# MECLabTUDA/Lifelong-nnUNet

Hardware: AMD Instinct MI355X
Metric: 3D patches/sec (whole node) + mean Dice vs ref, 5-level 3D Generic_UNet training step (higher is better)
Workload: dtype f16 (fp32 accumulate, fp32 master weights)

## Files before the change

lifelong-nnunet_amd/csrc/norm_act.hip:

```cpp
#include "igemm_common.h"

namespace {

constexpr int NT = 256;
typedef float float2v __attribute__((ext_vector_type(2)));
constexpr int MAX_BLOCKS = 1024;
constexpr int UNR = 4;

__device__ __forceinline__ half8 ld8(const half_t* p, int nt) {
    return nt ? __builtin_nontemporal_load(reinterpret_cast<const half8*>(p)) : *reinterpret_cast<const half8*>(p);
}
__device__ __forceinline__ void st8(half_t* p, const half8& v, int nt) {
    if (nt) __builtin_nontemporal_store(v, reinterpret_cast<half8*>(p));
    else *reinterpret_cast<half8*>(p) = v;
}
int in_nt_flag() {
    static int v = -1;
    if (v < 0) { const char* e = getenv("LNN_IN_NT"); v = (e && e[0] == '1') ? 1 : 0; }
    return v;
}

struct RowMap {
    int C8, VPB, c8, vl;
    bool active;
};
__device__ __forceinline__ RowMap row_map(int C) {
    RowMap r;
    r.C8 = C >> 3;
    r.VPB = NT / r.C8;
    r.c8 = threadIdx.x % r.C8;
    r.vl = threadIdx.x / r.C8;
    r.active = r.vl < r.VPB;
    return r;
}

__device__ __forceinline__ long vrange_len(long V, const RowMap& rm) {
    const long per = (V + gridDim.x - 1) / gridDim.x;
    return (per + rm.VPB - 1) / rm.VPB * rm.VPB;
}
__device__ __forceinline__ long vrange_begin(long V, const RowMap& rm) { return (long)blockIdx.x * vrange_len(V, rm); }
__device__ __forceinline__ long vrange_end(long V, const RowMap& rm) {
    const long e = vrange_begin(V, rm) + vrange_len(V, rm);
    return e < V ? e : V;
}

template <int NA, typename Sink>
__device__ __forceinline__ void block_channel_reduce(const RowMap& rm, int C, float (&part)[NA][8], float* red, Sink sink) {
    constexpr int W = NA * 8 + 1;
    __syncthreads();
    if (rm.active) {
#pragma unroll
        for (int a = 0; a < NA; ++a)
#pragma unroll
            for (int e = 0; e < 8; ++e) red[threadIdx.x * W + a * 8 + e] = part[a][e];
    }
    __syncthreads();
    for (int o = threadIdx.x; o < NA * C; o += NT) {
        const int a = o / C, c = o % C, c8 = c >> 3, e = c & 7;
        float s = 0.f;
        for (int vl = 0; vl < rm.VPB; ++vl) s += red[(vl * rm.C8 + c8) * W + a * 8 + e];
        sink(a, c, s);
    }
}

__global__ __launch_bounds__(NT) void in_stats_kernel(const half_t* __restrict__ y, long V, int C, float* pws) {
    __shared__ float red[NT * 17];
    const RowMap rm = row_map(C);
    const int n = blockIdx.y;
    const half_t* yn = y + (long)n * V * C;
    float part[2][8];
#pragma unroll
    for (int e = 0; e < 8; ++e) part[0][e] = part[1][e] = 0.f;
    if (rm.active) {
        const long end = vrange_end(V, rm), step = rm.VPB;
        long v = vrange_begin(V, rm) + rm.vl;
        const half_t* yp = yn + rm.c8 * 8;
        for (; v + (UNR - 1) * step < end; v += UNR * step) {
            half8 x[UNR];
#pragma unroll
            for (int u = 0; u < UNR; ++u) x[u] = *reinterpret_cast<const half8*>(yp + (v + u * step) * C);
#pragma unroll
            for (int u = 0; u < UNR; ++u)
#pragma unroll
                for (int e = 0; e < 8; ++e) {
                    const float f = (float)x[u][e];
                    part[0][e] += f;
                    part[1][e] += f * f;
                }
        }
        for (; v < end; v += step) {
            const half8 x = *reinterpret_cast<const half8*>(yp + v * C);
#pragma unroll
            for (int e = 0; e < 8; ++e) {
                const float f = (float)x[e];
                part[0][e] += f;
                part[1][e] += f * f;
            }
        }
    }
    block_channel_reduce<2>(rm, C, part, red, [&](int a, int c, float s) {
        pws[(((long)a * gridDim.x + blockIdx.x) * gridDim.y + n) * C + c] = s;
    });
}

constexpr int FSL = 64, FEB = 256 / FSL;
template <int SL>
__device__ __forceinline__ double slice_sum(const float* p, long stride, int nparts, int sl) {
    double acc = 0;
    int b = sl;
    for (; b + 15 * SL < nparts; b += 16 * SL) {
        float v[16];
#pragma unroll
        for (int k = 0; k < 16; ++k) v[k] = p[(long)(b + k * SL) * stride];
#pragma unroll
        for (int k = 0; k < 16; k += 4) acc += ((double)v[k] + (double)v[k + 1]) + ((double)v[k + 2] + (double)v[k + 3]);
    }
    for (; b + 3 * SL < nparts; b += 4 * SL) {
        const float a0 = p[(long)b * stride], a1 = p[(long)(b + SL) * stride], a2 = p[(long)(b + 2 * SL) * stride],
                    a3 = p[(long)(b + 3 * SL) * stride];
        acc += ((double)a0 + (double)a1) + ((double)a2 + (double)a3);
    }
    for (; b < nparts; b += SL) acc += (double)p[(long)b * stride];
    return acc;
}
template <int SL, int J>
__device__ __forceinline__ void reduce_slices(double (&s)[J], double* red) {
    constexpr int EB = 256 / SL;
    const int ii = threadIdx.x % EB, sl = threadIdx.x / EB;
    __syncthreads();
#pragma unroll
    for (int j = 0; j < J; ++j) red[j * 256 + threadIdx.x] = s[j];
    __syncthreads();
    if constexpr (SL > 16) {
        if (sl < 16) {
#pragma unroll
            for (int j = 0; j < J; ++j)
                for (int k = sl + 16; k < SL; k += 16) s[j] += red[j * 256 + k * EB + ii];
        }
        __syncthreads();
        if (sl < 16) {
#pragma unroll
            for (int j = 0; j < J; ++j) red[j * 256 + threadIdx.x] = s[j];
        }
        __syncthreads();
    }
    if (sl == 0) {
#pragma unroll
        for (int j = 0; j < J; ++j)
#pragma unroll
            for (int k = 1; k < 16; ++k) s[j] += red[j * 256 + k * EB + ii];
    }
}

__global__ void in_stats_finalize_kernel(const float* pws, int nblk, int NC, long V, float eps, float* mean, float* rstd) {
    __shared__ double red[2 * 256];
    const int ii = threadIdx.x % FEB, sl = threadIdx.x / FEB;
    const int i = blockIdx.x * FEB + ii;
    double t[2] = {0, 0};
    if (i < NC) {
        t[0] = slice_sum<FSL>(pws + i, NC, nblk, sl);
        t[1] = slice_sum<FSL>(pws + (long)nblk * NC + i, NC, nblk, sl);
    }
    reduce_slices<FSL, 2>(t, red);
    if (i >= NC || sl != 0) return;
    const double m = t[0] / (double)V;
    double var = t[1] / (double)V - m * m;
    if (var < 0) var = 0;
    mean[i] = (float)m;
    rstd[i] = (float)(1.0 / sqrt(var + (double)eps));
}

__global__ __launch_bounds__(NT) void in_lrelu_fwd_kernel(const half_t* __restrict__ y, half_t* __restrict__ z, int ld_z,
                                                          long V, int C, const float* __restrict__ mean,
                                                          const float* __restrict__ rstd, const float* __restrict__ gamma,
                                                          const float* __restrict__ beta, float slope, int nt) {
    const RowMap rm = row_map(C);
    if (!rm.active) return;
    const int n = blockIdx.y;
    float sc[8], sh[8];
#pragma unroll
    for (int e = 0; e < 8; ++e) {
        const int c = rm.c8 * 8 + e;
        sc[e] = gamma[c] * rstd[n * C + c];
        sh[e] = beta[c] - mean[n * C + c] * sc[e];
    }
    const half_t* yn = y + (long)n * V * C;
    half_t* zn = z + (long)n * V * ld_z;
    auto apply = [&](const half8& x) {
        half8 o;
#pragma unroll
        for (int e = 0; e < 8; ++e) {
            const float t = (float)x[e] * sc[e] + sh[e];
            o[e] = (half_t)(t > 0.f ? t : t * slope);
        }
        return o;
    };
    const long end = vrange_end(V, rm), step = rm.VPB;
    long v = vrange_begin(V, rm) + rm.vl;
    const half_t* yp = yn + rm.c8 * 8;
    half_t* zp = zn + rm.c8 * 8;
    for (; v + (UNR - 1) * step < end; v += UNR * step) {
        half8 x[UNR];
#pragma unroll
// ... 41 lines not shown
            const float zf = (float)o[e];
#pragma unroll
            for (int k = 0; k < KB; ++k) pk[k] += zf * w[k][e];
        }
        if (z) *reinterpret_cast<half8*>(zp + v * ld_z) = o;
        for (int m = 1; m < rm.C8; m <<= 1) {
#pragma unroll
            for (int k = 0; k < KB; ++k) pk[k] += __shfl_xor(pk[k], m, 64);
        }
        if (rm.c8 == 0) {
#pragma unroll
            for (int k = 0; k < KB; ++k)
                if (KT > 0 || k < K) {
                    if (stage) stage[k * (UNR * 64)] = pk[k];
                    else ln[(long)k * V + v] = pk[k];
                }
        }
    };
    long v = vrange_begin(V, rm) + rm.vl;
    if constexpr (STAGED) {
        const long run = (long)UNR * step;
        long base = vrange_begin(V, rm);
        int it = 0;
        for (; base + run <= end; base += run, ++it) {
            float* buf = lg + (it & 1) * (SEG_KMAX * UNR * 64);
            half8 x[UNR];
#pragma unroll
            for (int u = 0; u < UNR; ++u) x[u] = *reinterpret_cast<const half8*>(yp + (base + rm.vl + u * step) * C);
#pragma unroll
            for (int u = 0; u < UNR; ++u) one(x[u], base + rm.vl + u * step, buf + u * step + rm.vl);
            __syncthreads();
            const int q4 = (int)(run >> 2);
            for (int t = threadIdx.x; t < K * q4; t += NT) {
                const int k = t / q4, j = t - k * q4;
                *reinterpret_cast<floatx4*>(ln + (long)k * V + base + 4 * j) = *reinterpret_cast<const floatx4*>(buf + k * (UNR * 64) + 4 * j);
            }
        }
        v = base + rm.vl;
    } else {
        for (; v + (UNR - 1) * step < end; v += UNR * step) {
            half8 x[UNR];
#pragma unroll
            for (int u = 0; u < UNR; ++u) x[u] = *reinterpret_cast<const half8*>(yp + (v + u * step) * C);
#pragma unroll
            for (int u = 0; u < UNR; ++u) one(x[u], v + u * step, nullptr);
        }
    }
    for (; v < end; v += step) one(*reinterpret_cast<const half8*>(yp + v * C), v, nullptr);
}

__global__ __launch_bounds__(NT) void in_lrelu_bwd_reduce_kernel(const half_t* __restrict__ y, const half_t* __restrict__ dz,
                                                                 int ld_dz, long V, int C, const float* __restrict__ mean,
                                                                 const float* __restrict__ rstd, const float* __restrict__ gamma,
                                                                 const float* __restrict__ beta, float slope, float* pws, int nt) {
    __shared__ float red[NT * 17];
    const RowMap rm = row_map(C);
    const int n = blockIdx.y;
    float part[2][8];
#pragma unroll
    for (int e = 0; e < 8; ++e) part[0][e] = part[1][e] = 0.f;
    if (rm.active) {
        float mu[8], rs[8], ga[8], be[8];
#pragma unroll
        for (int e = 0; e < 8; ++e) {
            const int c = rm.c8 * 8 + e;
            mu[e] = mean[n * C + c]; rs[e] = rstd[n * C + c]; ga[e] = gamma[c]; be[e] = beta[c];
        }
        const half_t* yn = y + (long)n * V * C;
        const half_t* dzn = dz + (long)n * V * ld_dz;
        auto accum = [&](const half8& x, const half8& d) {
#pragma unroll
            for (int e = 0; e < 8; ++e) {
                const float xh = ((float)x[e] - mu[e]) * rs[e];
                const float pre = ga[e] * xh + be[e];
                const float g = (float)d[e] * (pre > 0.f ? 1.f : slope);
                part[0][e] += g;
                part[1][e] += g * xh;
            }
        };
        const long end = vrange_end(V, rm), step = rm.VPB;
        long v = vrange_begin(V, rm) + rm.vl;
        const half_t* yp = yn + rm.c8 * 8;
        const half_t* dp = dzn + rm.c8 * 8;
        constexpr int U2 = UNR / 2;
        for (; v + (U2 - 1) * step < end; v += U2 * step) {
            half8 x[U2], d[U2];
#pragma unroll
            for (int u = 0; u < U2; ++u) {
                x[u] = *reinterpret_cast<const half8*>(yp + (v + u * step) * C);
                d[u] = *reinterpret_cast<const half8*>(dp + (v + u * step) * ld_dz);
            }
#pragma unroll
            for (int u = 0; u < U2; ++u) accum(x[u], d[u]);
        }
        for (; v < end; v += step)
            accum(*reinterpret_cast<const half8*>(yp + v * C), *reinterpret_cast<const half8*>(dp + v * ld_dz));
    }
    block_channel_reduce<2>(rm, C, part, red, [&](int a, int c, float s) {
        pws[(((long)a * gridDim.x + blockIdx.x) * gridDim.y + n) * C + c] = s;
    });
}

__device__ __forceinline__ void in_bwd_sums_block(const float* pws, int nblk, int N, int C, int blk, double* red, double* ws,
                                                  float* dgamma, float* dbeta, float unscale, const float* raw_mean = nullptr,
                                                  const float* raw_rstd = nullptr) {
    const int ii = threadIdx.x % FEB, sl = threadIdx.x / FEB;
    const int c = blk * FEB + ii, NC = N * C;
    double g0 = 0, g1 = 0;
    for (int n = 0; n < N; n += 2) {
        const bool two = n + 1 < N;
        double o[4] = {0, 0, 0, 0};
        if (c < C) {
            const float* p0 = pws + n * C + c;
            o[0] = slice_sum<FSL>(p0, NC, nblk, sl);
            o[1] = slice_sum<FSL>(p0 + (long)nblk * NC, NC, nblk, sl);
            if (two) {
                o[2] = slice_sum<FSL>(p0 + C, NC, nblk, sl);
                o[3] = slice_sum<FSL>(p0 + C + (long)nblk * NC, NC, nblk, sl);
            }
        }
        reduce_slices<FSL, 4>(o, red);
        if (c < C && sl == 0) {
            const long i0 = (long)n * C + c;
            if (raw_mean) {
                o[1] = (double)raw_rstd[i0] * (o[1] - (double)raw_mean[i0] * o[0]);
                if (two) o[3] = (double)raw_rstd[i0 + C] * (o[3] - (double)raw_mean[i0 + C] * o[2]);
            }
            ws[i0 * 3 + 0] = o[0]; ws[i0 * 3 + 1] = o[1];
            g0 += o[0]; g1 += o[1];
            if (two) {
                ws[(i0 + C) * 3 + 0] = o[2]; ws[(i0 + C) * 3 + 1] = o[3];
                g0 += o[2]; g1 += o[3];
            }
        }
    }
    if (c >= C || sl != 0) return;
    if (dgamma) atomicAdd(dgamma + c, (float)(g1 * unscale));
    if (dbeta) atomicAdd(dbeta + c, (float)(g0 * unscale));
}
__global__ void in_lrelu_bwd_sums_kernel(const float* pws, int nblk, int NC, int C, double* ws, float* dgamma, float* dbeta,
                                         float unscale, const float* raw_mean, const float* raw_rstd) {
    __shared__ double red[4 * 256];
    in_bwd_sums_block(pws, nblk, NC / C, C, blockIdx.x, red, ws, dgamma, dbeta, unscale, raw_mean, raw_rstd);
}

template <bool DBIAS>
__global__ __launch_bounds__(NT) void in_lrelu_bwd_apply_kernel(half_t* __restrict__ y, const half_t* __restrict__ dz, int ld_dz,
                                                                long V, int C, const float* __restrict__ mean,
                                                                const float* __restrict__ rstd, const float* __restrict__ gamma,
                                                                const float* __restrict__ beta, float slope, const double* ws,
                                                                float* pws, int nt) {
    __shared__ float red[NT * 9];
    const RowMap rm = row_map(C);
// ... 58 lines not shown
    double t[1] = {i < N * C ? slice_sum<FSL>(pws + i, N * C, nblk, sl) : 0.0};
    reduce_slices<FSL, 1>(t, red);
    const double db = t[0];
    if (i >= N * C || sl != 0) return;
    const int c = i % C;
    (void)ws; (void)dgamma; (void)dbeta;
    if (dbias) atomicAdd(dbias + c, (float)(db * unscale));
}

template <int KT>
__device__ __forceinline__ void seg_dz(const float (&d)[KT], const float (&wr)[KT][8], const half8* prior, half8& dzh) {
#pragma unroll
    for (int e = 0; e < 8; ++e) {
        float o = 0.f;
#pragma unroll
        for (int k = 0; k < KT; ++k) o += d[k] * wr[k][e];
        if (prior) o += (float)(*prior)[e];
        dzh[e] = (half_t)o;
    }
}

template <int KT, bool QUAD>
struct DlFetch {
    float raw[QUAD ? 1 : KT];
    __device__ __forceinline__ void load(const float* __restrict__ dln, long V, long v) {
        if constexpr (QUAD) {
            const int kq = (int)(threadIdx.x & 3);
            raw[0] = dln[(long)(kq < KT ? kq : KT - 1) * V + v];
        } else {
#pragma unroll
            for (int k = 0; k < KT; ++k) raw[k] = dln[(long)k * V + v];
        }
    }
    __device__ __forceinline__ void get(float (&d)[KT]) const {
        if constexpr (QUAD) {
            const int r = __builtin_bit_cast(int, raw[0]);
            d[0] = __builtin_bit_cast(float, __builtin_amdgcn_mov_dpp(r, 0x00, 0xf, 0xf, true));
            if constexpr (KT > 1) d[1] = __builtin_bit_cast(float, __builtin_amdgcn_mov_dpp(r, 0x55, 0xf, 0xf, true));
            if constexpr (KT > 2) d[2] = __builtin_bit_cast(float, __builtin_amdgcn_mov_dpp(r, 0xaa, 0xf, 0xf, true));
            if constexpr (KT > 3) d[3] = __builtin_bit_cast(float, __builtin_amdgcn_mov_dpp(r, 0xff, 0xf, 0xf, true));
        } else {
#pragma unroll
            for (int k = 0; k < KT; ++k) d[k] = raw[k];
        }
    }
};

template <int KT, bool PRIOR, bool QUAD>
__global__ __launch_bounds__(NT, (KT <= 3 && !PRIOR && QUAD) ? 3 : 2) void in_lrelu_seg_bwd_reduce_kernel(const half_t* __restrict__ y, const half_t* __restrict__ dzp,
                                                                     int ld_dz, long V, int C, const float* __restrict__ mean,
                                                                     const float* __restrict__ rstd, const float* __restrict__ gamma,
                                                                     const float* __restrict__ beta, float slope,
                                                                     const float* __restrict__ segw, const float* __restrict__ dl,
                                                                     float* pws) {
    constexpr int NA = 2 + KT;
    __shared__ float red[NT * 17];
    const RowMap rm = row_map(C);
    const int n = blockIdx.y;
    float part[NA][8];
#pragma unroll
    for (int a = 0; a < NA; ++a)
#pragma unroll
        for (int e = 0; e < 8; ++e) part[a][e] = 0.f;
    if (rm.active) {
        float rs[8], nmr[8], sc[8], sh[8], wr[KT][8];
#pragma unroll
        for (int e = 0; e < 8; ++e) {
            const int c = rm.c8 * 8 + e;
            rs[e] = rstd[n * C + c];
            nmr[e] = -mean[n * C + c] * rs[e];
            sc[e] = gamma[c] * rs[e];
            sh[e] = beta[c] - mean[n * C + c] * sc[e];
#pragma unroll
            for (int k = 0; k < KT; ++k) wr[k][e] = segw[k * C + c];
        }
        const half_t* yp = y + (long)n * V * C + rm.c8 * 8;
        const half_t* dp = dzp + (long)n * V * ld_dz + rm.c8 * 8;
        const float* dln = dl + (long)n * KT * V;
        auto accum = [&](const half8& x, const half8& pr, const float (&d)[KT]) {
#pragma unroll
            for (int e = 0; e < 8; e += 2) {
                const float2v xf = {(float)x[e], (float)x[e + 1]};
                const float2v sc2 = {sc[e], sc[e + 1]}, sh2 = {sh[e], sh[e + 1]}, rs2 = {rs[e], rs[e + 1]}, nm2 = {nmr[e], nmr[e + 1]};
                const float2v t = xf * sc2 + sh2;
                const float2v sel = {t[0] > 0.f ? 1.f : slope, t[1] > 0.f ? 1.f : slope};
                const float2v z = t * sel;
                const float2v xh = xf * rs2 + nm2;
                float2v dz = {0.f, 0.f};
#pragma unroll
                for (int k = 0; k < KT; ++k) {
                    const float2v wk = {wr[k][e], wr[k][e + 1]};
                    dz += wk * d[k];
                }
                if (PRIOR) dz += float2v{(float)pr[e], (float)pr[e + 1]};
                const float2v g = dz * sel;
                float2v p0 = {part[0][e], part[0][e + 1]}, p1 = {part[1][e], part[1][e + 1]};
                p0 += g;
                p1 += g * xh;
                part[0][e] = p0[0]; part[0][e + 1] = p0[1];
                part[1][e] = p1[0]; part[1][e + 1] = p1[1];
#pragma unroll
                for (int k = 0; k < KT; ++k) {
                    float2v pk = {part[2 + k][e], part[2 + k][e + 1]};
                    pk += z * d[k];
                    part[2 + k][e] = pk[0]; part[2 + k][e + 1] = pk[1];
                }
            }
        };
        const long end = vrange_end(V, rm), step = rm.VPB;
        long v = vrange_begin(V, rm) + rm.vl;
        constexpr int U2 = (PRIOR || !QUAD) ? UNR / 2 : 3;
        for (; v + (U2 - 1) * step < end; v += U2 * step) {
            half8 x[U2], pr[U2];
            DlFetch<KT, QUAD> df[U2];
#pragma unroll
            for (int u = 0; u < U2; ++u) {
                x[u] = *reinterpret_cast<const half8*>(yp + (v + u * step) * C);
                if (PRIOR) pr[u] = *reinterpret_cast<const half8*>(dp + (v + u * step) * ld_dz);
                df[u].load(dln, V, v + u * step);
            }
#pragma unroll
            for (int u = 0; u < U2; ++u) {
                float d[KT];
                df[u].get(d);
                accum(x[u], pr[u], d);
            }
        }
        for (; v < end; v += step) {
            half8 pr;
            float d[KT];
            DlFetch<KT, QUAD> df;
            if (PRIOR) pr = *reinterpret_cast<const half8*>(dp + v * ld_dz);
            df.load(dln, V, v);
            df.get(d);
            accum(*reinterpret_cast<const half8*>(yp + v * C), pr, d);
        }
    }
    float* const pseg = pws + 2l * gridDim.x * gridDim.y * C;
#pragma unroll
    for (int a0 = 0; a0 < NA; a0 += 2) {
        float two[2][8];
#pragma unroll
        for (int e = 0; e < 8; ++e) {
            two[0][e] = part[a0][e];
            two[1][e] = a0 + 1 < NA ? part[a0 + 1 < NA ? a0 + 1 : a0][e] : 0.f;
        }
        block_channel_reduce<2>(rm, C, two, red, [&](int a, int c, float s) {
            const int aa = a0 + a;
            if (aa < 2) pws[(((long)aa * gridDim.x + blockIdx.x) * gridDim.y + n) * C + c] = s;
            else if (aa < NA) pseg[(((long)n * gridDim.x + blockIdx.x) * KT + (aa - 2)) * C + c] = s;
        });
    }
}

__global__ void in_lrelu_seg_bwd_sums_kernel(const float* pws, int nblk, int N, int C, int K, int nb_in, double* ws, float* dgamma,
                                             float* dbeta, float* dsegw, float unscale) {
    __shared__ double red[4 * 256];
    if ((int)blockIdx.x < nb_in) {
        in_bwd_sums_block(pws, nblk, N, C, blockIdx.x, red, ws, dgamma, dbeta, unscale);
        return;
    }
    const float* pseg = pws + 2l * nblk * N * C;
    const int ii = threadIdx.x % FEB, sl = threadIdx.x / FEB;
    const int i = (blockIdx.x - nb_in) * FEB + ii;
    double t[1] = {i < K * C ? slice_sum<FSL>(pseg + i, (long)K * C, nblk * N, sl) : 0.0};
    reduce_slices<FSL, 1>(t, red);
    if (sl == 0 && i < K * C) atomicAdd(dsegw + i, (float)(t[0] * unscale));
}

template <int KT, bool PRIOR, bool QUAD>
__global__ __launch_bounds__(NT) void in_lrelu_seg_bwd_apply_kernel(half_t* __restrict__ y, const half_t* __restrict__ dzp, int ld_dz,
                                                                    long V, int C, const float* __restrict__ mean,
                                                                    const float* __restrict__ rstd, const float* __restrict__ gamma,
                                                                    const float* __restrict__ beta, float slope,
                                                                    const float* __restrict__ segw, const float* __restrict__ dl,
                                                                    const double* ws) {
    const RowMap rm = row_map(C);
    if (!rm.active) return;
    const int n = blockIdx.y;
    float sc[8], sh[8], ca[8], cb[8], wr[KT][8];
    const float invV = 1.0f / (float)V;
#pragma unroll
    for (int e = 0; e < 8; ++e) {
        const int c = rm.c8 * 8 + e;
        const float rs = rstd[n * C + c], nmr = -mean[n * C + c] * rs;
        const float m1 = (float)(ws[((long)n * C + c) * 3 + 0] * (double)invV);
        const float m2 = (float)(ws[((long)n * C + c) * 3 + 1] * (double)invV);
        sc[e] = gamma[c] * rs;
        sh[e] = beta[c] - mean[n * C + c] * sc[e];
        ca[e] = -sc[e] * (m1 + nmr * m2);
        cb[e] = -sc[e] * rs * m2;
#pragma unroll
        for (int k = 0; k < KT; ++k) wr[k][e] = segw[k * C + c];
    }
    half_t* yp = y + (long)n * V * C + rm.c8 * 8;
    const half_t* dp = dzp + (long)n * V * ld_dz + rm.c8 * 8;
    const float* dln = dl + (long)n * KT * V;
    auto grad = [&](const half8& x, const half8& pr, const float (&d)[KT]) {
        half8 dzh, o;
        seg_dz<KT>(d, wr, PRIOR ? &pr : nullptr, dzh);
#pragma unroll
        for (int e = 0; e < 8; ++e) {
            const float xf = (float)x[e];
            const float t = xf * sc[e] + sh[e];
// ... 178 lines not shown
        }
        small_block_sum16(part, red, dtot);
        if (threadIdx.x < 64) {
            const double t = dtot[threadIdx.x];
            const int o = threadIdx.x >> 4, j = threadIdx.x & 15, c = blockIdx.x * 32 + o * 8 + (j & 7);
            bc[threadIdx.x] = (float)(t * (double)invV);
            gacc += t;
            if (c < C) ws[((long)n * C + c) * 3 + (j >> 3)] = t;
        }
        __syncthreads();
        if (chan_ok) {
            float m1[8], m2[8];
#pragma unroll
            for (int e = 0; e < 8; ++e) { m1[e] = bc[oc * 16 + e]; m2[e] = bc[oc * 16 + 8 + e]; }
            for (int r0 = rl; r0 < V; r0 += SU * SRL) {
                half8 xv[SU], gv[SU];
#pragma unroll
                for (int k = 0; k < SU; ++k) {
                    const int r = r0 + k * SRL, rc = r < V ? r : V - 1;
                    xv[k] = *reinterpret_cast<const half8*>(yn + rc * C);
                    gv[k] = *reinterpret_cast<const half8*>(dn + rc * ld_dz);
                }
#pragma unroll
                for (int k = 0; k < SU; ++k) {
                    half8 o;
#pragma unroll
                    for (int e = 0; e < 8; ++e) {
                        const float h = ((float)xv[k][e] - mu[e]) * rs[e];
                        const float pre = ga[e] * h + be[e];
                        const float gg = (float)gv[k][e] * (pre > 0.f ? 1.f : slope);
                        o[e] = (half_t)(ga[e] * rs[e] * (gg - m1[e] - h * m2[e]));
                    }
                    const int r = r0 + k * SRL;
                    if (r < V) *reinterpret_cast<half8*>(yn + r * C) = o;
                }
            }
        }
    }
    if (threadIdx.x < 64) {
        const int o = threadIdx.x >> 4, j = threadIdx.x & 15, c = blockIdx.x * 32 + o * 8 + (j & 7);
        if (c < C) {
            if (j < 8) { if (dbeta) atomicAdd(dbeta + c, (float)(gacc * unscale)); }
            else if (dgamma) atomicAdd(dgamma + c, (float)(gacc * unscale));
        }
    }
}

bool small_enabled() {
    static int v = -1;
    if (v < 0) { const char* e = getenv("LNN_IN_SMALL"); v = (e && e[0] == '0') ? 0 : 1; }
    return v != 0;
}

int blocks_for(long V, int C) {
    const int vpb = NT / (C / 8);
    long b = (V + (long)vpb * 8 - 1) / ((long)vpb * 8);
    if (b > MAX_BLOCKS) b = MAX_BLOCKS;
    if (b < 1) b = 1;
    return (int)b;
}

int check_common(const void* y, int N, long V, int C, const char* what) {
    LNN_REQUIRE(y != nullptr && lnn_aligned16(y), "%s: null/misaligned activation", what);
    LNN_REQUIRE(N > 0 && V > 0, "%s: bad dims", what);
    LNN_REQUIRE(C >= 8 && C % 8 == 0 && C <= 2048, "%s: channel count %d must be a multiple of 8 in [8, 2048]", what, C);
    return LNN_OK;
}

}

extern "C" int lnn_instnorm_small_volume(void) { return SMALL_V; }

int lnn_launch_in_small_fwd(hipStream_t s, const void* y, void* z, int ld_z, int N, long V, int C, float eps, const float* gamma,
                            const float* beta, float slope, float* mean, float* rstd) {
    if (int e = check_common(y, N, V, C, "lnn_conv3d_fwd_in_lrelu(norm)")) return e;
    LNN_REQUIRE(V <= SMALL_V, "lnn_conv3d_fwd_in_lrelu(norm): %ld voxels per sample exceed the single-launch limit %d", V, SMALL_V);
    LNN_REQUIRE(z != nullptr && lnn_aligned16(z) && ld_z >= C && ld_z % 8 == 0, "lnn_conv3d_fwd_in_lrelu(norm): bad z / ld_z");
    LNN_REQUIRE(mean && rstd && gamma && beta, "lnn_conv3d_fwd_in_lrelu(norm): null parameter");
    const dim3 grid(lnn_cdiv(C, 32), N);
    hipLaunchKernelGGL(in_small_fwd_kernel, grid, dim3(SNT), 0, s, (const half_t*)y, (half_t*)z, ld_z, (int)V, C, eps, gamma, beta, slope,
                       mean, rstd);
    LNN_CHECK_LAUNCH("lnn_conv3d_fwd_in_lrelu(norm)");
    return LNN_OK;
}

int lnn_launch_in_small_bwd(hipStream_t s, void* y, const void* dz, int ld_dz, int N, long V, int C, const float* mean, const float* rstd,
                            const float* gamma, const float* beta, float slope, double* ws, float* dgamma, float* dbeta, float unscale) {
    LNN_REQUIRE(V <= SMALL_V, "lnn_instnorm_lrelu_bwd(small): %ld voxels per sample exceed the single-launch limit %d", V, SMALL_V);
    hipLaunchKernelGGL(in_small_bwd_kernel, dim3(lnn_cdiv(C, 32)), dim3(SNT), 0, s, (half_t*)y, (const half_t*)dz, ld_dz, N, (int)V, C, mean,
                       rstd, gamma, beta, slope, ws, dgamma, dbeta, unscale);
    LNN_CHECK_LAUNCH("lnn_instnorm_lrelu_bwd(small)");
    return LNN_OK;
}

int lnn_launch_in_stats_finalize(hipStream_t s, const float* pws, int nslots, int N, int C, long V, float eps, float* mean, float* rstd) {
    hipLaunchKernelGGL(in_stats_finalize_kernel, dim3(lnn_cdiv(N * C, FEB)), dim3(256), 0, s, pws, nslots, N * C, V, eps, mean, rstd);
    LNN_CHECK_LAUNCH("lnn_instnorm_stats(finalize, fused partials)");
    return LNN_OK;
}

int lnn_launch_in_bwd_sums_raw(hipStream_t s, const float* pws, int nslots, int N, int C, const float* mean, const float* rstd,
                               double* ws, float* dgamma, float* dbeta, float unscale) {
    hipLaunchKernelGGL(in_lrelu_bwd_sums_kernel, dim3(lnn_cdiv(C, FEB)), dim3(256), 0, s, pws, nslots, N * C, C, ws, dgamma, dbeta,
                       unscale, mean, rstd);
    LNN_CHECK_LAUNCH("lnn_conv3d_dgrad_in_bwd_sums(sums)");
    return LNN_OK;
}

extern "C" size_t lnn_instnorm_ws_doubles(int N, int C) { return (size_t)N * C * 3 + (size_t)MAX_BLOCKS * N * C; }

extern "C" int lnn_instnorm_stats(lnn_stream_t s_, const void* y, int N, long V, int C, float eps, float* mean, float* rstd,
                                  double* ws) {
    hipStream_t s = (hipStream_t)s_;
    if (int e = check_common(y, N, V, C, "lnn_instnorm_stats")) return e;
    LNN_REQUIRE(mean && rstd && ws, "lnn_instnorm_stats: null output/workspace");
    float* pws = reinterpret_cast<float*>(ws + (size_t)N * C * 3);
    const int nblk = blocks_for(V, C);
    hipLaunchKernelGGL(in_stats_kernel, dim3(nblk, N), dim3(NT), 0, s, (const half_t*)y, V, C, pws);
    LNN_CHECK_LAUNCH("lnn_instnorm_stats");
    hipLaunchKernelGGL(in_stats_finalize_kernel, dim3(lnn_cdiv(N * C, FEB)), dim3(256), 0, s, pws, nblk, N * C, V, eps, mean, rstd);
    LNN_CHECK_LAUNCH("lnn_instnorm_stats(finalize)");
    return LNN_OK;
}

extern "C" int lnn_instnorm_lrelu_fwd(lnn_stream_t s_, const void* y, void* z, int ld_z, int N, long V, int C,
                                      const float* mean, const float* rstd, const float* gamma, const float* beta,
                                      float slope) {
    hipStream_t s = (hipStream_t)s_;
    if (int e = check_common(y, N, V, C, "lnn_instnorm_lrelu_fwd")) return e;
    LNN_REQUIRE(z != nullptr && lnn_aligned16(z) && ld_z >= C && ld_z % 8 == 0, "lnn_instnorm_lrelu_fwd: bad z / ld_z");
    LNN_REQUIRE(mean && rstd && gamma && beta, "lnn_instnorm_lrelu_fwd: null parameter");
    hipLaunchKernelGGL(in_lrelu_fwd_kernel, dim3(blocks_for(V, C), N), dim3(NT), 0, s, (const half_t*)y, (half_t*)z, ld_z,
                       V, C, mean, rstd, gamma, beta, slope, in_nt_flag());
    LNN_CHECK_LAUNCH("lnn_instnorm_lrelu_fwd");
    return LNN_OK;
}

extern "C" int lnn_instnorm_lrelu_seg_fwd(lnn_stream_t s_, const void* y, void* z, int ld_z, int N, long V, int C, const float* mean,
                                          const float* rstd, const float* gamma, const float* beta, float slope,
                                          const float* seg_w, float* logits, int K) {
    hipStream_t s = (hipStream_t)s_;
    if (int e = check_common(y, N, V, C, "lnn_instnorm_lrelu_seg_fwd")) return e;
    LNN_REQUIRE(z == nullptr || (lnn_aligned16(z) && ld_z >= C && ld_z % 8 == 0), "lnn_instnorm_lrelu_seg_fwd: bad z / ld_z");
    LNN_REQUIRE(mean && rstd && gamma && beta && seg_w && logits, "lnn_instnorm_lrelu_seg_fwd: null parameter");
    const int C8 = C >> 3;
    LNN_REQUIRE(K >= 1 && K <= SEG_KMAX && (C8 & (C8 - 1)) == 0 && C8 <= 64,
                "lnn_instnorm_lrelu_seg_fwd: K=%d / C=%d unsupported (K <= %d, C/8 a power of two <= 64): use lnn_instnorm_lrelu_fwd + lnn_seg1x1_fwd",
                K, C, SEG_KMAX);
    static int want_staged = -1;
    if (want_staged < 0) { const char* e = getenv("LNN_SEG_FWD_STAGED"); want_staged = (e && e[0] == '1') ? 1 : 0; }
    const bool staged = want_staged && C8 >= 4 && (V & 3) == 0 && lnn_aligned16(logits);
#define LNN_SF(ST, KT) hipLaunchKernelGGL((in_lrelu_seg_fwd_kernel<ST, KT>), dim3(blocks_for(V, C), N), dim3(NT), 0, s, (const half_t*)y, \
                                         (half_t*)z, ld_z, V, C, mean, rstd, gamma, beta, slope, seg_w, logits, K)
    if (staged) LNN_SF(true, 0);
    else if (K == 1) LNN_SF(false, 1);
    else if (K == 2) LNN_SF(false, 2);
    else if (K == 3) LNN_SF(false, 3);
    else if (K == 4) LNN_SF(false, 4);
    else LNN_SF(false, 0);
#undef LNN_SF
    LNN_CHECK_LAUNCH("lnn_instnorm_lrelu_seg_fwd");
    return LNN_OK;
}

extern "C" int lnn_instnorm_lrelu_bwd(lnn_stream_t s_, void* y, const void* dz, int ld_dz, int N, long V, int C,
                                      const float* mean, const float* rstd, const float* gamma, const float* beta,
                                      float slope, float* dgamma, float* dbeta, float* dbias, float grad_unscale,
                                      double* ws) {
    hipStream_t s = (hipStream_t)s_;
    if (int e = check_common(y, N, V, C, "lnn_instnorm_lrelu_bwd")) return e;
    LNN_REQUIRE(dz != nullptr && lnn_aligned16(dz) && ld_dz >= C && ld_dz % 8 == 0, "lnn_instnorm_lrelu_bwd: bad dz / ld_dz");
    LNN_REQUIRE(mean && rstd && gamma && beta && ws, "lnn_instnorm_lrelu_bwd: null parameter");
    if (V <= SMALL_V && !dbias && small_enabled())
        return lnn_launch_in_small_bwd(s, y, dz, ld_dz, N, V, C, mean, rstd, gamma, beta, slope, ws, dgamma, dbeta, grad_unscale);
    float* pws = reinterpret_cast<float*>(ws + (size_t)N * C * 3);
    const int nblk = blocks_for(V, C);
    const dim3 grid(nblk, N);
    hipLaunchKernelGGL(in_lrelu_bwd_reduce_kernel, grid, dim3(NT), 0, s, (const half_t*)y, (const half_t*)dz, ld_dz, V, C,
                       mean, rstd, gamma, beta, slope, pws, in_nt_flag());
    LNN_CHECK_LAUNCH("lnn_instnorm_lrelu_bwd(reduce)");
    hipLaunchKernelGGL(in_lrelu_bwd_sums_kernel, dim3(lnn_cdiv(C, FEB)), dim3(256), 0, s, pws, nblk, N * C, C, ws, dgamma, dbeta,
                       grad_unscale, (const float*)nullptr, (const float*)nullptr);
    LNN_CHECK_LAUNCH("lnn_instnorm_lrelu_bwd(sums)");
    if (dbias) {
        hipLaunchKernelGGL((in_lrelu_bwd_apply_kernel<true>), grid, dim3(NT), 0, s, (half_t*)y, (const half_t*)dz, ld_dz, V, C, mean,
                           rstd, gamma, beta, slope, ws, pws, in_nt_flag());
        LNN_CHECK_LAUNCH("lnn_instnorm_lrelu_bwd(apply)");
        hipLaunchKernelGGL(in_lrelu_bwd_finalize_kernel, dim3(lnn_cdiv(N * C, FEB)), dim3(256), 0, s, ws, pws, nblk, N, C, dgamma,
                           dbeta, dbias, grad_unscale);
        LNN_CHECK_LAUNCH("lnn_instnorm_lrelu_bwd(finalize)");
    } else {
        hipLaunchKernelGGL((in_lrelu_bwd_apply_kernel<false>), grid, dim3(NT), 0, s, (half_t*)y, (const half_t*)dz, ld_dz, V, C, mean,
                           rstd, gamma, beta, slope, ws, pws, in_nt_flag());
        LNN_CHECK_LAUNCH("lnn_instnorm_lrelu_bwd(apply)");
    }
    return LNN_OK;
}

extern "C" size_t lnn_instnorm_lrelu_seg_bwd_ws_doubles(int N, int C) { return (size_t)N * C * 3 + (size_t)MAX_BLOCKS * N * C * 3; }

extern "C" int lnn_instnorm_lrelu_seg_bwd(lnn_stream_t s_, void* y, const void* dz_prior, int ld_dz, const float* seg_w,
                                          const float* dlogits, float* seg_dw, int K, int N, long V, int C, const float* mean,
                                          const float* rstd, const float* gamma, const float* beta, float slope, float* dgamma,
                                          float* dbeta, float grad_unscale, double* ws) {
    hipStream_t s = (hipStream_t)s_;
    if (int e = check_common(y, N, V, C, "lnn_instnorm_lrelu_seg_bwd")) return e;
    LNN_REQUIRE(dz_prior == nullptr || (lnn_aligned16(dz_prior) && ld_dz >= C && ld_dz % 8 == 0),
                "lnn_instnorm_lrelu_seg_bwd: bad dz_prior / ld_dz");
    LNN_REQUIRE(mean && rstd && gamma && beta && ws && seg_w && dlogits && seg_dw, "lnn_instnorm_lrelu_seg_bwd: null parameter");
    LNN_REQUIRE(K >= 1 && K <= 4, "lnn_instnorm_lrelu_seg_bwd: K=%d unsupported (1..4): use lnn_seg1x1_bwd + lnn_instnorm_lrelu_bwd", K);
    float* pws = reinterpret_cast<float*>(ws + (size_t)N * C * 3);
    const int nblk = blocks_for(V, C);
    const dim3 grid(nblk, N);
    const half_t* pr = (const half_t*)dz_prior;
    const int nb_in = lnn_cdiv(C, FEB);
#define LNN_SB(KT, PRIOR) do { if (C % 32 == 0) LNN_SBQ(KT, PRIOR, true); else LNN_SBQ(KT, PRIOR, false); } while (0)
#define LNN_SBQ(KT, PRIOR, QUAD)                                                                                                     \
    do {                                                                                                                             \
        hipLaunchKernelGGL((in_lrelu_seg_bwd_reduce_kernel<KT, PRIOR, QUAD>), grid, dim3(NT), 0, s, (const half_t*)y, pr, ld_dz, V, C, \
                           mean, rstd, gamma, beta, slope, seg_w, dlogits, pws);                                                     \
        LNN_CHECK_LAUNCH("lnn_instnorm_lrelu_seg_bwd(reduce)");                                                                      \
        hipLaunchKernelGGL(in_lrelu_seg_bwd_sums_kernel, dim3(nb_in + lnn_cdiv(K * C, FEB)), dim3(256), 0, s, pws, nblk, N, C, K,     \
                           nb_in, ws, dgamma, dbeta, seg_dw, grad_unscale);                                                          \
        LNN_CHECK_LAUNCH("lnn_instnorm_lrelu_seg_bwd(sums)");                                                                        \
        hipLaunchKernelGGL((in_lrelu_seg_bwd_apply_kernel<KT, PRIOR, QUAD>), grid, dim3(NT), 0, s, (half_t*)y, pr, ld_dz, V, C, mean, \
                           rstd, gamma, beta, slope, seg_w, dlogits, ws);                                                            \
        LNN_CHECK_LAUNCH("lnn_instnorm_lrelu_seg_bwd(apply)");                                                                       \
    } while (0)
    if (pr) {
        if (K == 1) LNN_SB(1, true); else if (K == 2) LNN_SB(2, true); else if (K == 3) LNN_SB(3, true); else LNN_SB(4, true);
    } else {
        if (K == 1) LNN_SB(1, false); else if (K == 2) LNN_SB(2, false); else if (K == 3) LNN_SB(3, false); else LNN_SB(4, false);
    }
#undef LNN_SB
#undef LNN_SBQ
    return LNN_OK;
}

extern "C" int lnn_instnorm_lrelu_bwd_apply(lnn_stream_t s_, void* y, const void* dz, int ld_dz, int N, long V, int C,
                                            const float* mean, const float* rstd, const float* gamma, const float* beta, float slope,
                                            double* ws) {
    hipStream_t s = (hipStream_t)s_;
    if (int e = check_common(y, N, V, C, "lnn_instnorm_lrelu_bwd_apply")) return e;
    LNN_REQUIRE(dz != nullptr && lnn_aligned16(dz) && ld_dz >= C && ld_dz % 8 == 0, "lnn_instnorm_lrelu_bwd_apply: bad dz / ld_dz");
    LNN_REQUIRE(mean && rstd && gamma && beta && ws, "lnn_instnorm_lrelu_bwd_apply: null parameter");
    hipLaunchKernelGGL((in_lrelu_bwd_apply_kernel<false>), dim3(blocks_for(V, C), N), dim3(NT), 0, s, (half_t*)y, (const half_t*)dz, ld_dz,
                       V, C, mean, rstd, gamma, beta, slope, ws, (float*)nullptr, in_nt_flag());
    LNN_CHECK_LAUNCH("lnn_instnorm_lrelu_bwd_apply");
    return LNN_OK;
}

extern "C" int lnn_instnorm_lrelu_bwd_sums(lnn_stream_t s_, const void* y, const void* dz, int ld_dz, int N, long V, int C,
                                           const float* mean, const float* rstd, const float* gamma, const float* beta, float slope,
                                           float* dgamma, float* dbeta, float grad_unscale, double* ws) {
    hipStream_t s = (hipStream_t)s_;
    if (int e = check_common(y, N, V, C, "lnn_instnorm_lrelu_bwd_sums")) return e;
    LNN_REQUIRE(dz != nullptr && lnn_aligned16(dz) && ld_dz >= C && ld_dz % 8 == 0, "lnn_instnorm_lrelu_bwd_sums: bad dz / ld_dz");
    LNN_REQUIRE(mean && rstd && gamma && beta && ws, "lnn_instnorm_lrelu_bwd_sums: null parameter");
    float* pws = reinterpret_cast<float*>(ws + (size_t)N * C * 3);
    const int nblk = blocks_for(V, C);
    hipLaunchKernelGGL(in_lrelu_bwd_reduce_kernel, dim3(nblk, N), dim3(NT), 0, s, (const half_t*)y, (const half_t*)dz, ld_dz, V, C,
                       mean, rstd, gamma, beta, slope, pws, in_nt_flag());
    LNN_CHECK_LAUNCH("lnn_instnorm_lrelu_bwd_sums(reduce)");
    hipLaunchKernelGGL(in_lrelu_bwd_sums_kernel, dim3(lnn_cdiv(C, FEB)), dim3(256), 0, s, pws, nblk, N * C, C, ws, dgamma, dbeta,
                       grad_unscale, (const float*)nullptr, (const float*)nullptr);
    LNN_CHECK_LAUNCH("lnn_instnorm_lrelu_bwd_sums(sums)");
    return LNN_OK;
}
```

Before: 88.32.

## Fold instance-norm partial-sum finalization into reduce kernels via last-block tickets

Adds atomic ticket counters so the last blocks of each slice and then the final block of the stats and backward reduce kernels perform the cross-block fold. This lets the separate finalize and sums kernel launches be skipped by default. It removes one kernel launch and the dependency gap per instance-norm call, at the cost of threadfences, atomics and a serialized tail reduction done by single blocks. It also adds per-stream counter buffers and changes the workspace sizes.

```diff
diff --git a/lifelong-nnunet_amd/csrc/norm_act.hip b/lifelong-nnunet_amd/csrc/norm_act.hip
--- a/lifelong-nnunet_amd/csrc/norm_act.hip
+++ b/lifelong-nnunet_amd/csrc/norm_act.hip
@@ -1,4 +1,7 @@
 #include "igemm_common.h"
+#include <map>
+#include <mutex>
+#include <utility>
 
 namespace {
 
@@ -63,7 +66,140 @@
     }
 }
 
-__global__ __launch_bounds__(NT) void in_stats_kernel(const half_t* __restrict__ y, long V, int C, float* pws) {
+constexpr int FSL = 64, FEB = 256 / FSL;
+template <int SL>
+__device__ __forceinline__ double slice_sum(const float* p, long stride, int nparts, int sl) {
+    double acc = 0;
+    int b = sl;
+    for (; b + 15 * SL < nparts; b += 16 * SL) {
+        float v[16];
+#pragma unroll
+        for (int k = 0; k < 16; ++k) v[k] = p[(long)(b + k * SL) * stride];
+#pragma unroll
+        for (int k = 0; k < 16; k += 4) acc += ((double)v[k] + (double)v[k + 1]) + ((double)v[k + 2] + (double)v[k + 3]);
+    }
+    for (; b + 3 * SL < nparts; b += 4 * SL) {
+        const float a0 = p[(long)b * stride], a1 = p[(long)(b + SL) * stride], a2 = p[(long)(b + 2 * SL) * stride],
+                    a3 = p[(long)(b + 3 * SL) * stride];
+        acc += ((double)a0 + (double)a1) + ((double)a2 + (double)a3);
+    }
+    for (; b < nparts; b += SL) acc += (double)p[(long)b * stride];
+    return acc;
+}
+template <int SL, int J>
+__device__ __forceinline__ void reduce_slices(double (&s)[J], double* red) {
+    constexpr int EB = 256 / SL;
+    const int ii = threadIdx.x % EB, sl = threadIdx.x / EB;
+    __syncthreads();
+#pragma unroll
+    for (int j = 0; j < J; ++j) red[j * 256 + threadIdx.x] = s[j];
+    __syncthreads();
+    if constexpr (SL > 16) {
+        if (sl < 16) {
+#pragma unroll
+            for (int j = 0; j < J; ++j)
+                for (int k = sl + 16; k < SL; k += 16) s[j] += red[j * 256 + k * EB + ii];
+        }
+        __syncthreads();
+        if (sl < 16) {
+#pragma unroll
+            for (int j = 0; j < J; ++j) red[j * 256 + threadIdx.x] = s[j];
+        }
+        __syncthreads();
+    }
+    if (sl == 0) {
+#pragma unroll
+        for (int j = 0; j < J; ++j)
+#pragma unroll
+            for (int k = 1; k < 16; ++k) s[j] += red[j * 256 + k * EB + ii];
+    }
+}
+
+constexpr int FOLD_A = 0, FOLD_B = FSL, FOLD_FINAL = 2 * FSL, FOLD_CTRS = 2 * FSL + 1;
+struct Fold {
+    unsigned* ctr;
+    double* sws;
+};
+
+__device__ __forceinline__ bool fold_last_ticket(unsigned* ctr, unsigned expected) {
+    __shared__ unsigned drawn;
+    __threadfence();
+    __syncthreads();
+    if (threadIdx.x == 0) {
+        const unsigned t = atomicAdd(ctr, 1u);
+        if (t == expected - 1) atomicExch(ctr, 0u);
+        drawn = t;
+    }
+    __syncthreads();
+    const bool last = drawn == expected - 1;
+    if (last) __threadfence();
+    return last;
+}
+__device__ __forceinline__ unsigned fold_rows_of_slice(int nrows, int sl) { return sl < nrows ? (unsigned)((nrows - sl + FSL - 1) / FSL) : 0u; }
+
+__device__ __forceinline__ bool fold_slice_totals(unsigned* ctr, unsigned* fin, int other_slices, int row, int nrows, int per_row,
+                                                  const float* part, const float* part2, long stride, int nent, double* sws) {
+    const int sl = row % FSL;
+    if (!fold_last_ticket(ctr + sl, fold_rows_of_slice(nrows, sl) * (unsigned)per_row)) return false;
+    for (int e = threadIdx.x; e < (part2 ? 2 * nent : nent); e += blockDim.x)
+        sws[(long)e * FSL + sl] = e < nent ? slice_sum<FSL>(part + e, stride, nrows, sl) : slice_sum<FSL>(part2 + (e - nent), stride, nrows, sl);
+    return fold_last_ticket(fin, (unsigned)((nrows < FSL ? nrows : FSL) + other_slices));
+}
+
+__device__ __forceinline__ double fold_entry_stage1(const double* sws, long e, int nrows, int q) {
+    const double* p = sws + e * FSL;
+    double v[FSL / 16];
+#pragma unroll
+    for (int j = 0; j < FSL / 16; ++j) v[j] = q + 16 * j < nrows ? p[q + 16 * j] : 0.0;
+    double s = v[0];
+#pragma unroll
+    for (int j = 1; j < FSL / 16; ++j) s += v[j];
+    return s;
+}
+__device__ __forceinline__ double fold_entry_stage2(double s) {
+    const int base = (threadIdx.x & 63) & ~15;
+    double t = __shfl(s, base, 64);
+#pragma unroll
+    for (int k = 1; k < 16; ++k) t += __shfl(s, base + k, 64);
+    return t;
+}
+
+__device__ __forceinline__ void fold_stats_final(const double* sws, int nrows, int NC, long V, float eps, float* mean, float* rstd) {
+    const int q = threadIdx.x & 15, per = blockDim.x >> 4;
+    for (int i0 = 0; i0 < NC; i0 += per) {
+        const int i = i0 + (threadIdx.x >> 4), ic = i < NC ? i : NC - 1;
+        const double s0 = fold_entry_stage1(sws, ic, nrows, q), s1 = fold_entry_stage1(sws, (long)NC + ic, nrows, q);
+        const double t[2] = {fold_entry_stage2(s0), fold_entry_stage2(s1)};
+        if (i >= NC || q != 0) continue;
+        const double m = t[0] / (double)V;
+        double var = t[1] / (double)V - m * m;
+        if (var < 0) var = 0;
+        mean[i] = (float)m;
+        rstd[i] = (float)(1.0 / sqrt(var + (double)eps));
+    }
+}
+
+__device__ __forceinline__ void fold_bwd_sums_final(const double* sws, int nrows, int N, int C, double* ws, float* dgamma, float* dbeta,
+                                                    float unscale) {
+    const int q = threadIdx.x & 15, per = blockDim.x >> 4, NC = N * C;
+    for (int c0 = 0; c0 < C; c0 += per) {
+        const int c = c0 + (threadIdx.x >> 4), cc = c < C ? c : C - 1;
+        double g0 = 0, g1 = 0;
+        for (int n = 0; n < N; ++n) {
+            const long i0 = (long)n * C + cc;
+            const double s0 = fold_entry_stage1(sws, i0, nrows, q), s1 = fold_entry_stage1(sws, (long)NC + i0, nrows, q);
+            const double o0 = fold_entry_stage2(s0), o1 = fold_entry_stage2(s1);
+            if (c < C && q == 0) { ws[i0 * 3 + 0] = o0; ws[i0 * 3 + 1] = o1; }
+            g0 += o0; g1 += o1;
+        }
+        if (c >= C || q != 0) continue;
+        if (dgamma) atomicAdd(dgamma + c, (float)(g1 * unscale));
+        if (dbeta) atomicAdd(dbeta + c, (float)(g0 * unscale));
+    }
+}
+
+__global__ __launch_bounds__(NT) void in_stats_kernel(const half_t* __restrict__ y, long V, int C, float* pws, Fold fold, float eps,
+                                                      float* mean, float* rstd) {
     __shared__ float red[NT * 17];
     const RowMap rm = row_map(C);
     const int n = blockIdx.y;
@@ -101,54 +237,18 @@
     block_channel_reduce<2>(rm, C, part, red, [&](int a, int c, float s) {
         pws[(((long)a * gridDim.x + blockIdx.x) * gridDim.y + n) * C + c] = s;
     });
-}
-
-constexpr int FSL = 64, FEB = 256 / FSL;
-template <int SL>
-__device__ __forceinline__ double slice_sum(const float* p, long stride, int nparts, int sl) {
-    double acc = 0;
-    int b = sl;
-    for (; b + 15 * SL < nparts; b += 16 * SL) {
-        float v[16];
-#pragma unroll
-        for (int k = 0; k < 16; ++k) v[k] = p[(long)(b + k * SL) * stride];
-#pragma unroll
-        for (int k = 0; k < 16; k += 4) acc += ((double)v[k] + (double)v[k + 1]) + ((double)v[k + 2] + (double)v[k + 3]);
-    }
-    for (; b + 3 * SL < nparts; b += 4 * SL) {
-        const float a0 = p[(long)b * stride], a1 = p[(long)(b + SL) * stride], a2 = p[(long)(b + 2 * SL) * stride],
-                    a3 = p[(long)(b + 3 * SL) * stride];
-        acc += ((double)a0 + (double)a1) + ((double)a2 + (double)a3);
-    }
-    for (; b < nparts; b += SL) acc += (double)p[(long)b * stride];
-    return acc;
-}
-template <int SL, int J>
-__device__ __forceinline__ void reduce_slices(double (&s)[J], double* red) {
-    constexpr int EB = 256 / SL;
-    const int ii = threadIdx.x % EB, sl = threadIdx.x / EB;
-    __syncthreads();
-#pragma unroll
-    for (int j = 0; j < J; ++j) red[j * 256 + threadIdx.x] = s[j];
-    __syncthreads();
-    if constexpr (SL > 16) {
-        if (sl < 16) {
-#pragma unroll
-            for (int j = 0; j < J; ++j)
-                for (int k = sl + 16; k < SL; k += 16) s[j] += red[j * 256 + k * EB + ii];
-        }
-        __syncthreads();
-        if (sl < 16) {
-#pragma unroll
-            for (int j = 0; j < J; ++j) red[j * 256 + threadIdx.x] = s[j];
-        }
-        __syncthreads();
-    }
-    if (sl == 0) {
-#pragma unroll
-        for (int j = 0; j < J; ++j)
-#pragma unroll
-            for (int k = 1; k < 16; ++k) s[j] += red[j * 256 + k * EB + ii];
+    if (!fold.ctr) return;
+    const int nblk = gridDim.x, NC = gridDim.y * C;
+    if (fold_slice_totals(fold.ctr + FOLD_A, fold.ctr + FOLD_FINAL, 0, blockIdx.x, nblk, gridDim.y, pws, pws + (long)nblk * NC, NC, NC, fold.sws))
+        fold_stats_final(fold.sws, nblk, NC, V, eps, mean, rstd);
+}
+
+__device__ __forceinline__ void fold_segw_final(const double* sws, int nrows, int nent, float* dsegw, float unscale) {
+    const int q = threadIdx.x & 15, per = blockDim.x >> 4;
+    for (int i0 = 0; i0 < nent; i0 += per) {
+        const int i = i0 + (threadIdx.x >> 4);
+        const double t = fold_entry_stage2(fold_entry_stage1(sws, i < nent ? i : nent - 1, nrows, q));
+        if (i < nent && q == 0) atomicAdd(dsegw + i, (float)(t * unscale));
     }
 }
 
@@ -296,7 +396,8 @@
 __global__ __launch_bounds__(NT) void in_lrelu_bwd_reduce_kernel(const half_t* __restrict__ y, const half_t* __restrict__ dz,
                                                                  int ld_dz, long V, int C, const float* __restrict__ mean,
                                                                  const float* __restrict__ rstd, const float* __restrict__ gamma,
-                                                                 const float* __restrict__ beta, float slope, float* pws, int nt) {
+                                                                 const float* __restrict__ beta, float slope, float* pws, int nt,
+                                                                 Fold fold, double* ws, float* dgamma, float* dbeta, float unscale) {
     __shared__ float red[NT * 17];
     const RowMap rm = row_map(C);
     const int n = blockIdx.y;
@@ -343,6 +444,10 @@
     block_channel_reduce<2>(rm, C, part, red, [&](int a, int c, float s) {
         pws[(((long)a * gridDim.x + blockIdx.x) * gridDim.y + n) * C + c] = s;
     });
+    if (!fold.ctr) return;
+    const int nblk = gridDim.x, NC = gridDim.y * C;
+    if (fold_slice_totals(fold.ctr + FOLD_A, fold.ctr + FOLD_FINAL, 0, blockIdx.x, nblk, gridDim.y, pws, pws + (long)nblk * NC, NC, NC, fold.sws))
+        fold_bwd_sums_final(fold.sws, nblk, gridDim.y, C, ws, dgamma, dbeta, unscale);
 }
 
 __device__ __forceinline__ void in_bwd_sums_block(const float* pws, int nblk, int N, int C, int blk, double* red, double* ws,
@@ -507,7 +612,8 @@
                                                                      const float* __restrict__ rstd, const float* __restrict__ gamma,
                                                                      const float* __restrict__ beta, float slope,
                                                                      const float* __restrict__ segw, const float* __restrict__ dl,
-                                                                     float* pws) {
+                                                                     float* pws, Fold fold, double* ws, float* dgamma, float* dbeta,
+                                                                     float* dsegw, float unscale) {
     constexpr int NA = 2 + KT;
     __shared__ float red[NT * 17];
     const RowMap rm = row_map(C);
@@ -605,6 +711,16 @@
             if (aa < 2) pws[(((long)aa * gridDim.x + blockIdx.x) * gridDim.y + n) * C + c] = s;
             else if (aa < NA) pseg[(((long)n * gridDim.x + blockIdx.x) * KT + (aa - 2)) * C + c] = s;
         });
+    }
+    if (!fold.ctr) return;
+    const int nblk = gridDim.x, N = gridDim.y, NC = N * C;
+    const int nsl_in = nblk < FSL ? nblk : FSL, nsl_seg = nblk * N < FSL ? nblk * N : FSL;
+    double* const sws_seg = fold.sws + 2l * NC * FSL;
+    fold_slice_totals(fold.ctr + FOLD_A, fold.ctr + FOLD_FINAL, nsl_seg, blockIdx.x, nblk, N, pws, pws + (long)nblk * NC, NC, NC, fold.sws);
+    if (fold_slice_totals(fold.ctr + FOLD_B, fold.ctr + FOLD_FINAL, nsl_in, n * nblk + blockIdx.x, nblk * N, 1, pseg, nullptr, (long)KT * C,
+                          KT * C, sws_seg)) {
+        fold_bwd_sums_final(fold.sws, nblk, N, C, ws, dgamma, dbeta, unscale);
+        fold_segw_final(sws_seg, nblk * N, KT * C, dsegw, unscale);
     }
 }
 
@@ -889,6 +1005,30 @@
     return v != 0;
 }
 
+bool fold_enabled() {
+    static int v = -1;
+    if (v < 0) { const char* e = getenv("LNN_IN_FOLD"); v = (e && e[0] == '0') ? 0 : 1; }
+    return v != 0;
+}
+
+unsigned* fold_counters(hipStream_t s) {
+    if (!fold_enabled()) return nullptr;
+    static std::mutex mu;
+    static std::map<std::pair<int, hipStream_t>, unsigned*> sets;
+    int dev = 0;
+    if (hipGetDevice(&dev) != hipSuccess) return nullptr;
+    std::lock_guard<std::mutex> lock(mu);
+    auto it = sets.find({dev, s});
+    if (it != sets.end()) return it->second;
+    unsigned* p = nullptr;
+    if (hipMalloc(&p, FOLD_CTRS * sizeof(unsigned)) != hipSuccess) { (void)hipGetLastError(); return nullptr; }
+    if (hipMemsetAsync(p, 0, FOLD_CTRS * sizeof(unsigned), s) != hipSuccess) { (void)hipGetLastError(); (void)hipFree(p); return nullptr; }
+    sets[{dev, s}] = p;
+    return p;
+}
+constexpr size_t FOLD_WS_IN = (size_t)2 * FSL;
+constexpr size_t WS_PART_IN = MAX_BLOCKS, WS_PART_SEG = (size_t)MAX_BLOCKS * 3;
+
 int blocks_for(long V, int C) {
     const int vpb = NT / (C / 8);
     long b = (V + (long)vpb * 8 - 1) / ((long)vpb * 8);
@@ -944,7 +1084,7 @@
     return LNN_OK;
 }
 
-extern "C" size_t lnn_instnorm_ws_doubles(int N, int C) { return (size_t)N * C * 3 + (size_t)MAX_BLOCKS * N * C; }
+extern "C" size_t lnn_instnorm_ws_doubles(int N, int C) { return (size_t)N * C * (3 + WS_PART_IN + FOLD_WS_IN); }
 
 extern "C" int lnn_instnorm_stats(lnn_stream_t s_, const void* y, int N, long V, int C, float eps, float* mean, float* rstd,
                                   double* ws) {
@@ -953,8 +1093,10 @@
     LNN_REQUIRE(mean && rstd && ws, "lnn_instnorm_stats: null output/workspace");
     float* pws = reinterpret_cast<float*>(ws + (size_t)N * C * 3);
     const int nblk = blocks_for(V, C);
-    hipLaunchKernelGGL(in_stats_kernel, dim3(nblk, N), dim3(NT), 0, s, (const half_t*)y, V, C, pws);
+    const Fold fold{fold_counters(s), ws + (size_t)N * C * (3 + WS_PART_IN)};
+    hipLaunchKernelGGL(in_stats_kernel, dim3(nblk, N), dim3(NT), 0, s, (const half_t*)y, V, C, pws, fold, eps, mean, rstd);
     LNN_CHECK_LAUNCH("lnn_instnorm_stats");
+    if (fold.ctr) return LNN_OK;
     hipLaunchKernelGGL(in_stats_finalize_kernel, dim3(lnn_cdiv(N * C, FEB)), dim3(256), 0, s, pws, nblk, N * C, V, eps, mean, rstd);
     LNN_CHECK_LAUNCH("lnn_instnorm_stats(finalize)");
     return LNN_OK;
@@ -1013,12 +1155,15 @@
     float* pws = reinterpret_cast<float*>(ws + (size_t)N * C * 3);
     const int nblk = blocks_for(V, C);
     const dim3 grid(nblk, N);
+    const Fold fold{fold_counters(s), ws + (size_t)N * C * (3 + WS_PART_IN)};
     hipLaunchKernelGGL(in_lrelu_bwd_reduce_kernel, grid, dim3(NT), 0, s, (const half_t*)y, (const half_t*)dz, ld_dz, V, C,
-                       mean, rstd, gamma, beta, slope, pws, in_nt_flag());
+                       mean, rstd, gamma, beta, slope, pws, in_nt_flag(), fold, ws, dgamma, dbeta, grad_unscale);
     LNN_CHECK_LAUNCH("lnn_instnorm_lrelu_bwd(reduce)");
-    hipLaunchKernelGGL(in_lrelu_bwd_sums_kernel, dim3(lnn_cdiv(C, FEB)), dim3(256), 0, s, pws, nblk, N * C, C, ws, dgamma, dbeta,
-                       grad_unscale, (const float*)nullptr, (const float*)nullptr);
-    LNN_CHECK_LAUNCH("lnn_instnorm_lrelu_bwd(sums)");
+    if (!fold.ctr) {
+        hipLaunchKernelGGL(in_lrelu_bwd_sums_kernel, dim3(lnn_cdiv(C, FEB)), dim3(256), 0, s, pws, nblk, N * C, C, ws, dgamma, dbeta,
+                           grad_unscale, (const float*)nullptr, (const float*)nullptr);
+        LNN_CHECK_LAUNCH("lnn_instnorm_lrelu_bwd(sums)");
+    }
     if (dbias) {
         hipLaunchKernelGGL((in_lrelu_bwd_apply_kernel<true>), grid, dim3(NT), 0, s, (half_t*)y, (const half_t*)dz, ld_dz, V, C, mean,
                            rstd, gamma, beta, slope, ws, pws, in_nt_flag());
@@ -1034,7 +1179,9 @@
     return LNN_OK;
 }
 
-extern "C" size_t lnn_instnorm_lrelu_seg_bwd_ws_doubles(int N, int C) { return (size_t)N * C * 3 + (size_t)MAX_BLOCKS * N * C * 3; }
+extern "C" size_t lnn_instnorm_lrelu_seg_bwd_ws_doubles(int N, int C) {
+    return (size_t)N * C * (3 + WS_PART_SEG + FOLD_WS_IN) + (size_t)FSL * 4 * C;
+}
 
 extern "C" int lnn_instnorm_lrelu_seg_bwd(lnn_stream_t s_, void* y, const void* dz_prior, int ld_dz, const float* seg_w,
                                           const float* dlogits, float* seg_dw, int K, int N, long V, int C, const float* mean,
@@ -1051,15 +1198,18 @@
     const dim3 grid(nblk, N);
     const half_t* pr = (const half_t*)dz_prior;
     const int nb_in = lnn_cdiv(C, FEB);
+    const Fold fold{fold_counters(s), ws + (size_t)N * C * (3 + WS_PART_SEG)};
 #define LNN_SB(KT, PRIOR) do { if (C % 32 == 0) LNN_SBQ(KT, PRIOR, true); else LNN_SBQ(KT, PRIOR, false); } while (0)
 #define LNN_SBQ(KT, PRIOR, QUAD)                                                                                                     \
     do {                                                                                                                             \
         hipLaunchKernelGGL((in_lrelu_seg_bwd_reduce_kernel<KT, PRIOR, QUAD>), grid, dim3(NT), 0, s, (const half_t*)y, pr, ld_dz, V, C, \
-                           mean, rstd, gamma, beta, slope, seg_w, dlogits, pws);                                                     \
+                           mean, rstd, gamma, beta, slope, seg_w, dlogits, pws, fold, ws, dgamma, dbeta, seg_dw, grad_unscale);      \
         LNN_CHECK_LAUNCH("lnn_instnorm_lrelu_seg_bwd(reduce)");                                                                      \
-        hipLaunchKernelGGL(in_lrelu_seg_bwd_sums_kernel, dim3(nb_in + lnn_cdiv(K * C, FEB)), dim3(256), 0, s, pws, nblk, N, C, K,     \
-                           nb_in, ws, dgamma, dbeta, seg_dw, grad_unscale);                                                          \
-        LNN_CHECK_LAUNCH("lnn_instnorm_lrelu_seg_bwd(sums)");                                                                        \
+        if (!fold.ctr) {                                                                                                             \
+            hipLaunchKernelGGL(in_lrelu_seg_bwd_sums_kernel, dim3(nb_in + lnn_cdiv(K * C, FEB)), dim3(256), 0, s, pws, nblk, N, C, K, \
+                               nb_in, ws, dgamma, dbeta, seg_dw, grad_unscale);                                                      \
+            LNN_CHECK_LAUNCH("lnn_instnorm_lrelu_seg_bwd(sums)");                                                                    \
+        }                                                                                                                            \
         hipLaunchKernelGGL((in_lrelu_seg_bwd_apply_kernel<KT, PRIOR, QUAD>), grid, dim3(NT), 0, s, (half_t*)y, pr, ld_dz, V, C, mean, \
                            rstd, gamma, beta, slope, seg_w, dlogits, ws);                                                            \
         LNN_CHECK_LAUNCH("lnn_instnorm_lrelu_seg_bwd(apply)");                                                                       \
@@ -1096,9 +1246,11 @@
     LNN_REQUIRE(mean && rstd && gamma && beta && ws, "lnn_instnorm_lrelu_bwd_sums: null parameter");
     float* pws = reinterpret_cast<float*>(ws + (size_t)N * C * 3);
     const int nblk = blocks_for(V, C);
+    const Fold fold{fold_counters(s), ws + (size_t)N * C * (3 + WS_PART_IN)};
     hipLaunchKernelGGL(in_lrelu_bwd_reduce_kernel, dim3(nblk, N), dim3(NT), 0, s, (const half_t*)y, (const half_t*)dz, ld_dz, V, C,
-                       mean, rstd, gamma, beta, slope, pws, in_nt_flag());
+                       mean, rstd, gamma, beta, slope, pws, in_nt_flag(), fold, ws, dgamma, dbeta, grad_unscale);
     LNN_CHECK_LAUNCH("lnn_instnorm_lrelu_bwd_sums(reduce)");
+    if (fold.ctr) return LNN_OK;
     hipLaunchKernelGGL(in_lrelu_bwd_sums_kernel, dim3(lnn_cdiv(C, FEB)), dim3(256), 0, s, pws, nblk, N * C, C, ws, dgamma, dbeta,
                        grad_unscale, (const float*)nullptr, (const float*)nullptr);
     LNN_CHECK_LAUNCH("lnn_instnorm_lrelu_bwd_sums(sums)");
```

Result: slower. 74.49 (-15.7%).
